# BraveGroup/DCD

Hardware: AMD Instinct MI355X
Metric: images/sec DGDE train step (bs=8, 384x1280) (higher is better)
Workload: dtype f32; 1 GPU; DGDE train bs=8 fp32 on 1xMI355X, synthetic KITTI 384x1280 + random kpts_ann (DGDE.yaml, DLA-34+DCNv2, 6 objects/image); global_batch=8, per_gpu_batch=8, input=384x1280, parallelism=dp1, dcn_precision=f32, step_launch=eager, sync_bn=False

## Files before the change

### dcd_amd/csrc/conv.hip

```cpp
#include <hip/hip_runtime.h>
#include <stdint.h>
#include <stdlib.h>

#include "../../include/dcd_hip.h"
#include "tuning_env.h"
#include "lds_limit.h"
#include "bf16_split.h"

typedef float f32x16 __attribute__((ext_vector_type(16)));
typedef float f32x4 __attribute__((ext_vector_type(4)));
typedef float f32x2 __attribute__((ext_vector_type(2)));

namespace {

constexpr int WN_CH = 8;
constexpr int WN_NT = 512;

template <int TR, int TC, int NB>
struct WinoGeom {
    static constexpr int KS = 32 * NB;
    static constexpr int U = 16 * KS * WN_CH;
    static constexpr int NTILE = TR * TC;
    static constexpr int ROWS = 4 * TR + 2;
    static constexpr int Q = (2 * TC + 8) / 4;
    static constexpr int RS = TC == 16 ? 48 : 42;
    static constexpr int PLANE = ROWS * RS;
    static constexpr int IN = WN_CH * PLANE;
    static constexpr int BUF = IN + U;
    static_assert(NTILE <= 32 && 4 * Q <= RS && RS % 2 == 0 && (2 * TC) % 4 == 0, "region geometry");
};

__device__ __forceinline__ void win_read4(const float *e, float (&q)[4])
{
    const f32x2 a = *reinterpret_cast<const f32x2 *>(e), b = *reinterpret_cast<const f32x2 *>(e + 2),
                c = *reinterpret_cast<const f32x2 *>(e + 4);
    q[0] = a.y; q[1] = b.x; q[2] = b.y; q[3] = c.x;
}

template <int RS>
__device__ __forceinline__ void win_store4(float *d, const f32x4 v)
{
    if constexpr (RS % 4 == 0) {
        *reinterpret_cast<f32x4 *>(d) = v;
    } else {
        *reinterpret_cast<f32x2 *>(d) = f32x2{v.x, v.y};
        *reinterpret_cast<f32x2 *>(d + 2) = f32x2{v.z, v.w};
    }
}

__device__ __forceinline__ void xcd_remap(int &bx, int &by)
{
    const int gx = gridDim.x, NT = gx * gridDim.y;
    const int L = bx + gx * by;
    const int xc = L & 7, slot = L >> 3;
    const int q = NT >> 3, r = NT & 7;
    const int Lp = (xc < r ? xc * (q + 1) : r * (q + 1) + (xc - r) * q) + slot;
    by = Lp / gx;
    bx = Lp - by * gx;
}

__device__ __forceinline__ void wino_prep_body(const float *__restrict__ w, float *__restrict__ ul, int Cc, int Kk, int mode, int nchunk,
                                               int nz, int WN_KS, int first, int step)
{
    const int n = nz * nchunk * WN_KS * WN_CH;
    for (int idx = first; idx < n; idx += step) {
        int r = idx;
        const int s = r & 3; r >>= 2;
        const int h = r & 1; r >>= 1;
        const int kk = r % WN_KS; r /= WN_KS;
        const int ck = r % nchunk, z = r / nchunk;
        const int k = z * WN_KS + kk, c = ck * WN_CH + 2 * s + h;
        float g[3][3];
#pragma unroll
        for (int a = 0; a < 3; ++a)
#pragma unroll
            for (int b = 0; b < 3; ++b) {
                float v = 0.f;
                if (k < Kk && c < Cc)
                    v = mode == 0 ? w[(((size_t)k * Cc + c) * 3 + a) * 3 + b] : w[(((size_t)c * Kk + k) * 3 + (2 - a)) * 3 + (2 - b)];
                g[a][b] = v;
            }
        float t[4][3];
#pragma unroll
        for (int b = 0; b < 3; ++b) {
            t[0][b] = g[0][b];
            t[1][b] = 0.5f * (g[0][b] + g[1][b] + g[2][b]);
            t[2][b] = 0.5f * (g[0][b] - g[1][b] + g[2][b]);
            t[3][b] = g[2][b];
        }
#pragma unroll
        for (int xi = 0; xi < 4; ++xi) {
            const float u[4] = {t[xi][0], 0.5f * (t[xi][0] + t[xi][1] + t[xi][2]), 0.5f * (t[xi][0] - t[xi][1] + t[xi][2]), t[xi][2]};
#pragma unroll
            for (int nu = 0; nu < 4; ++nu)
                ul[((((size_t)(z * nchunk + ck) * 16 + xi * 4 + nu) * 2 + h) * WN_KS + kk) * 4 + s] = u[nu];
        }
    }
}

__global__ void wino_prep_weights(const float *__restrict__ w, float *__restrict__ ul, int Cc, int Kk, int mode, int nchunk, int nz,
                                  int WN_KS)
{
    wino_prep_body(w, ul, Cc, Kk, mode, nchunk, nz, WN_KS, blockIdx.x * blockDim.x + threadIdx.x, gridDim.x * blockDim.x);
}

struct PrepBoth {
    float *ul[2];
    int Cc[2], Kk[2], nchunk[2], nz[2], ks[2];
};

__global__ void wino_prep_weights_both(const float *__restrict__ w, PrepBoth p)
{
    const int mode = blockIdx.y;
    if (!p.ul[mode]) return;
    wino_prep_body(w, p.ul[mode], p.Cc[mode], p.Kk[mode], mode, p.nchunk[mode], p.nz[mode], p.ks[mode],
                   blockIdx.x * blockDim.x + threadIdx.x, gridDim.x * blockDim.x);
}

__global__ void wino_prep_weights_table(const long long *__restrict__ table)
{
    const long long *e = table + 5 * (size_t)blockIdx.z;
    const float *w = reinterpret_cast<const float *>(e[0]);
    const int mode = blockIdx.y;
    float *ul = reinterpret_cast<float *>(e[1 + mode]);
    if (!w || !ul) return;
    const int Cin = (int)e[3], Cout = (int)e[4];
    const int Cc = mode ? Cout : Cin, Kk = mode ? Cin : Cout;
    const int WN_KS = Kk <= 32 ? 32 : 64;
    wino_prep_body(w, ul, Cc, Kk, mode, (Cc + WN_CH - 1) / WN_CH, (Kk + WN_KS - 1) / WN_KS, WN_KS,
                   blockIdx.x * blockDim.x + threadIdx.x, gridDim.x * blockDim.x);
}

template <int TR, int TC, int NB>
__global__ __launch_bounds__(WN_NT) void wino_conv3x3_f32(const float *__restrict__ x, const float *__restrict__ ul, float *y,
                                                          float *__restrict__ part, const float *__restrict__ bias,
                                                          const float *residual, int Cc, int H, int W, int Kk, int tiles_x,
                                                          int nchunk, int nz)
{
    using G = WinoGeom<TR, TC, NB>;
    constexpr int WN_ROWS = G::ROWS, WN_RS = G::RS, WN_PLANE = G::PLANE, WN_IN = G::IN, WN_BUF = G::BUF, WN_Q = G::Q;
    constexpr int WN_KS = G::KS, WN_U = G::U;
    extern __shared__ __attribute__((aligned(16))) float lds[];
    const int tid = threadIdx.x;
    const int lane = tid & 63, wave = tid >> 6;
    const int p = lane & 31, h = lane >> 5;
    const int xi = wave & 3, tg = wave >> 2;
    int bx = blockIdx.x, b = blockIdx.y;
    xcd_remap(bx, b);
    const int ty = bx / tiles_x, tx = bx - ty * tiles_x;
    const int r0 = ty * (4 * TR), c0 = tx * (2 * TC);
    const int z = blockIdx.z % nz, ks = blockIdx.z / nz, ksplit = gridDim.z / nz;
    const int ck0 = (int)((int64_t)ks * nchunk / ksplit), ck1 = (int)((int64_t)(ks + 1) * nchunk / ksplit);
    const int HW = H * W;
    const bool live = p < G::NTILE;
    const int pe = live ? p : 0;
    const int trow = pe / TC, tcol = pe - trow * TC;

    const int ra = xi == 0 ? 0 : 1, rb = xi == 3 ? 3 : 2;
    const float sa = xi == 2 ? -1.f : 1.f, sb = (xi == 0 || xi == 3) ? -1.f : 1.f;
    const int lanebase = (2 * TR * tg + 2 * trow) * WN_RS + 2 + 2 * tcol + h * WN_PLANE;
    const int base1 = lanebase + ra * WN_RS, base2 = lanebase + rb * WN_RS;

    const float *x_b = x + (size_t)b * Cc * HW;
    const float *ul_z = ul + (size_t)z * nchunk * WN_U;

    constexpr int KIN = (WN_CH * WN_ROWS * WN_Q + WN_NT - 1) / WN_NT;
    constexpr int KW = WN_U / 4 / WN_NT;
    int sg[KIN], sl[KIN];
    bool sv_[KIN];
#pragma unroll
    for (int k = 0; k < KIN; ++k) {
        const int e = tid + WN_NT * k;
        const int ch = e / (WN_ROWS * WN_Q), rem = e - ch * (WN_ROWS * WN_Q);
        const int row = rem / WN_Q, q = rem - row * WN_Q;
        const int yy = r0 - 1 + row, xx = c0 - 4 + 4 * q;
        sv_[k] = e < WN_CH * WN_ROWS * WN_Q;
        sg[k] = (sv_[k] && yy >= 0 && yy < H && xx >= 0 && xx < W) ? ch * HW + yy * W + xx : -1;
        sl[k] = ch * WN_PLANE + row * WN_RS + 4 * q;
    }
    f32x4 rin[KIN];
    auto issue_w = [&](int ck, float *buf) {
        const float *src = ul_z + (size_t)ck * WN_U + 4 * tid;
        float *dst = buf + WN_IN + 4 * 64 * __builtin_amdgcn_readfirstlane(wave);
#pragma unroll
        for (int k = 0; k < KW; ++k)
            __builtin_amdgcn_global_load_lds(src + 4 * WN_NT * k, (__attribute__((address_space(3))) void *)(dst + 4 * WN_NT * k), 16, 0, 0);
    };
    auto issue = [&](int ck) {
        const float *src = x_b + (size_t)ck * WN_CH * HW;
        const int cleft = Cc - ck * WN_CH;
#pragma unroll
        for (int k = 0; k < KIN; ++k) {
            const f32x4 zero4 = {0.f, 0.f, 0.f, 0.f};
            rin[k] = zero4;
            if (sv_[k] && sg[k] >= 0 && (tid + WN_NT * k) / (WN_ROWS * WN_Q) < cleft) rin[k] = *reinterpret_cast<const f32x4 *>(src + sg[k]);
        }
    };
    auto commit = [&](float *buf) {
#pragma unroll
        for (int k = 0; k < KIN; ++k)
            if (sv_[k]) win_store4<WN_RS>(buf + sl[k], rin[k]);
    };

    f32x16 acc[4][NB];
#pragma unroll
    for (int nu = 0; nu < 4; ++nu)
#pragma unroll
        for (int mb = 0; mb < NB; ++mb)
#pragma unroll
            for (int r = 0; r < 16; ++r) acc[nu][mb][r] = 0.f;

    issue_w(ck0, lds);
    issue(ck0);
    commit(lds);
    asm volatile("s_waitcnt vmcnt(0)" ::: "memory");
    __syncthreads();

    for (int ck = ck0; ck < ck1; ++ck) {
        const float *buf = lds + ((ck - ck0) & 1) * WN_BUF;
#ifndef WN_ABL_NOSTAGE
        if (ck + 1 < ck1) {
            issue_w(ck + 1, lds + ((ck + 1 - ck0) & 1) * WN_BUF);
            issue(ck + 1);
        }
#endif
        const float *ub = buf + WN_IN + ((xi * 4 * 2 + h) * WN_KS + p) * 4;
        const float *cp1 = buf + base1, *cp2 = buf + base2;
        f32x4 a0[4], a1[4];
#pragma unroll
        for (int nu = 0; nu < 4; ++nu) {
            a0[nu] = *reinterpret_cast<const f32x4 *>(ub + (nu * WN_KS) * 8);
            if (NB == 2) a1[nu] = *reinterpret_cast<const f32x4 *>(ub + (nu * WN_KS) * 8 + 32 * 4);
        }
        float qa[4], qb[4];
#ifndef WN_ABL_NOLDS
        win_read4(cp1, qa);
        win_read4(cp2, qb);
#endif
#pragma unroll
        for (int s = 0; s < 4; ++s) {
#ifdef WN_ABL_NOLDS
            const float t0 = sa * (float)s, t1 = sb, t2 = sa + sb, t3 = (float)ck;
#else
            const float t0 = sa * qa[0] + sb * qb[0], t1 = sa * qa[1] + sb * qb[1];
            const float t2 = sa * qa[2] + sb * qb[2], t3 = sa * qa[3] + sb * qb[3];
            if (s + 1 < 4) {
                win_read4(cp1 + 2 * (s + 1) * WN_PLANE, qa);
                win_read4(cp2 + 2 * (s + 1) * WN_PLANE, qb);
            }
#endif
            const float v[4] = {t0 - t2, t1 + t2, t2 - t1, t1 - t3};
            __builtin_amdgcn_sched_barrier(0);
#pragma unroll
            for (int nu = 0; nu < 4; ++nu) {
                acc[nu][0] = __builtin_amdgcn_mfma_f32_32x32x2f32(a0[nu][s], v[nu], acc[nu][0], 0, 0, 0);
                if (NB == 2) acc[nu][NB - 1] = __builtin_amdgcn_mfma_f32_32x32x2f32(a1[nu][s], v[nu], acc[nu][NB - 1], 0, 0, 0);
            }
        }
#ifndef WN_ABL_NOSTAGE
        if (ck + 1 < ck1) commit(lds + ((ck + 1 - ck0) & 1) * WN_BUF);
#endif
        asm volatile("s_waitcnt vmcnt(0)" ::: "memory");
        __syncthreads();
    }
#ifdef WN_ABL_NOEPI
    if (acc[0][0][0] != 123.456f) return;
#endif

    float *ex = lds;
    float *y_b = (ks == 0 ? y : part + (size_t)(ks - 1) * gridDim.y * Kk * HW) + (size_t)b * Kk * HW;
    const float *r_b = (residual && ks == 0) ? residual + (size_t)b * Kk * HW : nullptr;
    const int orow0 = r0 + 2 * TR * tg + 2 * trow, ocol = c0 + 2 * tcol;
#pragma unroll
    for (int mb = 0; mb < NB; ++mb) {
        float *mine = ex + (size_t)wave * 32 * 64 + lane;
#pragma unroll
        for (int r = 0; r < 16; ++r) {
            mine[r * 64] = acc[0][mb][r] + acc[1][mb][r] + acc[2][mb][r];
            mine[(16 + r) * 64] = acc[1][mb][r] - acc[2][mb][r] - acc[3][mb][r];
        }
        __syncthreads();
        const float *t0 = ex + (size_t)(tg * 4 + 0) * 32 * 64 + lane, *t1 = t0 + 32 * 64, *t2 = t1 + 32 * 64, *t3 = t2 + 32 * 64;
        if (live && ocol < W) {
#pragma unroll
            for (int rr = 0; rr < 4; ++rr) {
                const int r = 4 * xi + rr;
                const int k = z * WN_KS + mb * 32 + (r & 3) + 8 * (r >> 2) + 4 * h;
                const float a0 = t0[r * 64], a1 = t1[r * 64], a2 = t2[r * 64], a3 = t3[r * 64];
                const float b0 = t0[(16 + r) * 64], b1 = t1[(16 + r) * 64], b2 = t2[(16 + r) * 64], b3 = t3[(16 + r) * 64];
                if (k < Kk) {
                    const float bk = (bias && ks == 0) ? bias[k] : 0.f;
                    const size_t o = (size_t)k * HW + (size_t)orow0 * W + ocol;
                    float *dst = y_b + o;
                    f32x2 r0 = {bk, bk}, r1 = {bk, bk};
                    if (r_b) {
                        if (orow0 < H) r0 += *reinterpret_cast<const f32x2 *>(r_b + o);
                        if (orow0 + 1 < H) r1 += *reinterpret_cast<const f32x2 *>(r_b + o + W);
                    }
                    if (orow0 < H) *reinterpret_cast<f32x2 *>(dst) = f32x2{a0 + a1 + a2 + r0.x, b0 + b1 + b2 + r0.y};
                    if (orow0 + 1 < H) *reinterpret_cast<f32x2 *>(dst + W) = f32x2{a1 - a2 - a3 + r1.x, b1 - b2 - b3 + r1.y};
                }
            }
        }
        __syncthreads();
    }
}

constexpr int WS_CH = 16;

template <int NB>
__device__ __forceinline__ void wino_prep_split_body(const float *__restrict__ w, unsigned *__restrict__ us, int Cc, int Kk, int mode,
                                                     int nchunk, int nz, int first, int step)
{
    constexpr int KS = 32 * NB;
    const int n = nz * nchunk * KS * 2 * 4;
    for (int idx = first; idx < n; idx += step) {
        int r = idx;
        const int d = r & 3; r >>= 2;
        const int h = r & 1; r >>= 1;
        const int kk = r % KS; r /= KS;
        const int ck = r % nchunk, z = r / nchunk;
        const int k = z * KS + kk;
        float u[2][16];
#pragma unroll
        for (int e = 0; e < 2; ++e) {
            const int c = ck * WS_CH + 2 * (2 * d + e) + h;
            float g[3][3];
#pragma unroll
            for (int a = 0; a < 3; ++a)
#pragma unroll
                for (int b = 0; b < 3; ++b) {
                    float v = 0.f;
                    if (k < Kk && c < Cc)
                        v = mode == 0 ? w[(((size_t)k * Cc + c) * 3 + a) * 3 + b] : w[(((size_t)c * Kk + k) * 3 + (2 - a)) * 3 + (2 - b)];
                    g[a][b] = v;
                }
            float t[4][3];
#pragma unroll
            for (int b = 0; b < 3; ++b) {
                t[0][b] = g[0][b];
                t[1][b] = 0.5f * (g[0][b] + g[1][b] + g[2][b]);
                t[2][b] = 0.5f * (g[0][b] - g[1][b] + g[2][b]);
                t[3][b] = g[2][b];
            }
#pragma unroll
            for (int xi = 0; xi < 4; ++xi) {
                u[e][xi * 4 + 0] = t[xi][0];
                u[e][xi * 4 + 1] = 0.5f * (t[xi][0] + t[xi][1] + t[xi][2]);
                u[e][xi * 4 + 2] = 0.5f * (t[xi][0] - t[xi][1] + t[xi][2]);
                u[e][xi * 4 + 3] = t[xi][2];
            }
        }
        const int ob = kk >> 5, lane = h * 32 + (kk & 31);
        unsigned *dst = us + (size_t)(z * nchunk + ck) * (16 * NB * 2 * 256);
#pragma unroll
        for (int pos = 0; pos < 16; ++pos) {
            unsigned hi, lo;
            sp_split_pair(u[0][pos], u[1][pos], hi, lo);
            dst[((pos * NB + ob) * 2 + 0) * 256 + lane * 4 + d] = hi;
            dst[((pos * NB + ob) * 2 + 1) * 256 + lane * 4 + d] = lo;
        }
    }
}

#include "conv_direct_bf16.inc"
#include "conv1x1_bf16.inc"
#include "conv1x1_f32.inc"
#include "conv_s2_f32.inc"

template <int NB>
__global__ void wino_prep_weights_split(const float *__restrict__ w, unsigned *__restrict__ us, int Cc, int Kk, int mode, int nchunk,
                                        int nz)
{
    wino_prep_split_body<NB>(w, us, Cc, Kk, mode, nchunk, nz, blockIdx.x * blockDim.x + threadIdx.x, gridDim.x * blockDim.x);
}

__global__ void wino_prep_weights_split_table(const long long *__restrict__ table)
{
    const long long *e = table + 5 * (size_t)blockIdx.z;
    const float *w = reinterpret_cast<const float *>(e[0]);
    const int mode = blockIdx.y;
    unsigned *us = reinterpret_cast<unsigned *>(e[1 + mode]);
    if (!w || !us) return;
    const int Cin = (int)e[3], Cout = (int)e[4];
    const int Cc = mode ? Cout : Cin, Kk = mode ? Cin : Cout;
    const int nb = Kk <= 32 ? 1 : 2, nchunk = (Cc + WS_CH - 1) / WS_CH, nz = (Kk + 32 * nb - 1) / (32 * nb);
    const int first = blockIdx.x * blockDim.x + threadIdx.x, step = gridDim.x * blockDim.x;
    if (nb == 2) wino_prep_split_body<2>(w, us, Cc, Kk, mode, nchunk, nz, first, step);
    else wino_prep_split_body<1>(w, us, Cc, Kk, mode, nchunk, nz, first, step);
}

template <int NB, int NP>
__global__ __launch_bounds__(WN_NT) void wino_conv3x3_split(const float *__restrict__ x, const unsigned *__restrict__ us, float *y,
                                                            float *__restrict__ part, const float *__restrict__ bias,
                                                            const float *residual, int Cc, int H, int W, int Kk, int tiles_x,
                                                            int nchunk, int nz)
{
    constexpr int TR = 2, TC = 16;
    using G = WinoGeom<TR, TC, NB>;
    constexpr int WN_ROWS = G::ROWS, WN_RS = G::RS, WN_PLANE = G::PLANE, WN_Q = G::Q, WN_KS = G::KS;
    constexpr int WIN = (WS_CH * WN_PLANE + 3) & ~3;
    constexpr int WSLAB = 16 * NB * 2 * 256;
    extern __shared__ __attribute__((aligned(16))) float lds[];
    float *win = lds;
    unsigned *wbuf = reinterpret_cast<unsigned *>(lds + WIN);
    const int tid = threadIdx.x;
    const int lane = tid & 63, wave = __builtin_amdgcn_readfirstlane(tid >> 6);
    const int p = lane & 31, h = lane >> 5;
    const int xi = wave & 3, tg = wave >> 2;
    int bx = blockIdx.x, b = blockIdx.y;
    xcd_remap(bx, b);
    const int ty = bx / tiles_x, tx = bx - ty * tiles_x;
    const int r0 = ty * (4 * TR), c0 = tx * (2 * TC);
    const int z = blockIdx.z % nz, ks = blockIdx.z / nz, ksplit = gridDim.z / nz;
    const int ck0 = (int)((int64_t)ks * nchunk / ksplit), ck1 = (int)((int64_t)(ks + 1) * nchunk / ksplit);
    const int HW = H * W;
    const int trow = p / TC, tcol = p - trow * TC;

    const int ra = xi == 0 ? 0 : 1, rb = xi == 3 ? 3 : 2;
    const float sa = xi == 2 ? -1.f : 1.f, sb = (xi == 0 || xi == 3) ? -1.f : 1.f;
    const int lanebase = (2 * TR * tg + 2 * trow) * WN_RS + 2 + 2 * tcol + h * WN_PLANE;
    const int base1 = lanebase + ra * WN_RS, base2 = lanebase + rb * WN_RS;

    const float *x_b = x + (size_t)b * Cc * HW;
    const unsigned *us_z = us + (size_t)z * nchunk * WSLAB;

    constexpr int NITEM = WS_CH * WN_ROWS * WN_Q;
    constexpr int KIN = (NITEM + WN_NT - 1) / WN_NT;
    int sg[KIN], sl[KIN];
#pragma unroll
    for (int k = 0; k < KIN; ++k) {
        const int e = tid + WN_NT * k;
        const int ch = e / (WN_ROWS * WN_Q), rem = e - ch * (WN_ROWS * WN_Q);
        const int row = rem / WN_Q, q = rem - row * WN_Q;
        const int yy = r0 - 1 + row, xx = c0 - 4 + 4 * q;
        const bool ok = e < NITEM && yy >= 0 && yy < H && xx >= 0 && xx < W;
        sg[k] = ok ? ch * HW + yy * W + xx : -1;
        sl[k] = e < NITEM ? ch * WN_PLANE + row * WN_RS + 4 * q : -1;
    }
    f32x4 rin[KIN];
    auto issue_in = [&](int ck) {
        const float *src = x_b + (size_t)ck * WS_CH * HW;
        const int cleft = Cc - ck * WS_CH;
#pragma unroll
        for (int k = 0; k < KIN; ++k) {
            const f32x4 zero4 = {0.f, 0.f, 0.f, 0.f};
            rin[k] = zero4;
            if (sg[k] >= 0 && (tid + WN_NT * k) / (WN_ROWS * WN_Q) < cleft) rin[k] = *reinterpret_cast<const f32x4 *>(src + sg[k]);
        }
    };
    auto commit_in = [&]() {
#pragma unroll
        for (int k = 0; k < KIN; ++k)
// ... 291 lines not shown
    if (t0 < t1) {
        issue(t0);
        commit(lds);
        if (t0 + 1 < t1) issue(t0 + 1);
    }
    __syncthreads();
    for (int t = t0; t < t1; ++t) {
        const float *bw = lds + ((t - t0) & 1) * WW_BUF;
        float *nb = lds + (((t - t0) & 1) ^ 1) * WW_BUF;
        const float *ia = bw + lane_in + ra * WW_IROW, *ib = bw + lane_in + rb * WW_IROW;
        const float *d0 = bw + WW_IN + lane_dy, *d1 = d0 + (NOB - 1) * 32 * WW_DPLANE;
#ifdef WW_ABL_NOLDS
        float u0 = sa, u1 = sb;
#else
        const f32x2 pa0 = *reinterpret_cast<const f32x2 *>(ia), pa1 = *reinterpret_cast<const f32x2 *>(ia + 2);
        const f32x2 pb0 = *reinterpret_cast<const f32x2 *>(ib), pb1 = *reinterpret_cast<const f32x2 *>(ib + 2);
        f32x2 ca = *reinterpret_cast<const f32x2 *>(ia + 4), cb2 = *reinterpret_cast<const f32x2 *>(ib + 4);
        float u0 = sa * pa0.y + sb * pb0.y, u1 = sa * pa1.x + sb * pb1.x;
        float qa2 = pa1.y, qa3 = ca.x, qb2 = pb1.y, qb3 = cb2.x;
        f32x2 g00 = *reinterpret_cast<const f32x2 *>(d0), g01 = *reinterpret_cast<const f32x2 *>(d0 + 32);
        f32x2 g10 = *reinterpret_cast<const f32x2 *>(d1), g11 = *reinterpret_cast<const f32x2 *>(d1 + 32);
#endif
        float ev[12];
        sp_u32x2 pk[12];
#pragma unroll
        for (int s = 0; s < 8; ++s) {
#ifndef WW_ABL_NOSTAGE
            if (s == 4 && t + 1 < t1) {
                commit(nb);
                if (t + 2 < t1) issue(t + 2);
            }
#endif
#ifdef WW_ABL_NOLDS
            const float u2 = sa + (float)t, u3 = sb * (float)s;
            const float a0 = ea * (float)t, a1 = eb, b0 = ea + (float)s, b1 = eb * (float)s;
#else
            const float u2 = sa * qa2 + sb * qb2, u3 = sa * qa3 + sb * qb3;
            const float a0 = ea * g00.x + eb * g01.x, a1 = ea * g00.y + eb * g01.y;
            const float b0 = ea * g10.x + eb * g11.x, b1 = ea * g10.y + eb * g11.y;
            if (s + 1 < 8) {
                qa2 = ca.y; qb2 = cb2.y;
                ca = *reinterpret_cast<const f32x2 *>(ia + 2 * s + 6); cb2 = *reinterpret_cast<const f32x2 *>(ib + 2 * s + 6);
                qa3 = ca.x; qb3 = cb2.x;
                g00 = *reinterpret_cast<const f32x2 *>(d0 + 2 * s + 2); g01 = *reinterpret_cast<const f32x2 *>(d0 + 2 * s + 34);
                g10 = *reinterpret_cast<const f32x2 *>(d1 + 2 * s + 2); g11 = *reinterpret_cast<const f32x2 *>(d1 + 2 * s + 34);
            }
#endif
            const float v[4] = {u0 - u2, u1 + u2, u2 - u1, u1 - u3};
            const float wa[4] = {a0, a0 + a1, a0 - a1, -a1};
            const float wb[4] = {b0, b0 + b1, b0 - b1, -b1};
            if constexpr (BF) {
#pragma unroll
                for (int nu = 0; nu < 4; ++nu) {
                    if (s & 1) {
                        pk[nu][(s >> 1) & 1] = __builtin_bit_cast(unsigned, __builtin_convertvector(sp_f32x2{ev[nu], v[nu]}, sp_bf16x2));
                        pk[4 + nu][(s >> 1) & 1] = __builtin_bit_cast(unsigned, __builtin_convertvector(sp_f32x2{ev[4 + nu], wa[nu]}, sp_bf16x2));
                        if (NOB == 2) pk[8 + nu][(s >> 1) & 1] = __builtin_bit_cast(unsigned, __builtin_convertvector(sp_f32x2{ev[8 + nu], wb[nu]}, sp_bf16x2));
                    } else {
                        ev[nu] = v[nu]; ev[4 + nu] = wa[nu]; ev[8 + nu] = wb[nu];
                    }
                }
                if ((s & 3) == 3) {
#pragma unroll
                    for (int nu = 0; nu < 4; ++nu) {
                        const sp_s16x4 bv = __builtin_bit_cast(sp_s16x4, pk[nu]);
                        acc[nu][0] = __builtin_amdgcn_mfma_f32_32x32x8bf16_1k(__builtin_bit_cast(sp_s16x4, pk[4 + nu]), bv, acc[nu][0], 0, 0, 0);
                        if (NOB == 2)
                            acc[nu][NOB - 1] = __builtin_amdgcn_mfma_f32_32x32x8bf16_1k(__builtin_bit_cast(sp_s16x4, pk[8 + nu]), bv, acc[nu][NOB - 1], 0, 0, 0);
                    }
                }
            } else {
                __builtin_amdgcn_sched_barrier(0);
#pragma unroll
                for (int nu = 0; nu < 4; ++nu) {
                    acc[nu][0] = __builtin_amdgcn_mfma_f32_32x32x2f32(wa[nu], v[nu], acc[nu][0], 0, 0, 0);
                    if (NOB == 2) acc[nu][NOB - 1] = __builtin_amdgcn_mfma_f32_32x32x2f32(wb[nu], v[nu], acc[nu][NOB - 1], 0, 0, 0);
                }
            }
            u0 = u2;
            u1 = u3;
        }

#ifndef WW_ABL_NOBAR
        __syncthreads();
#endif
    }

#ifdef WW_ABL_NOEPI
    if (acc[0][0][0] != 123.456f) return;
#endif
    float *mine = part + ((size_t)blk * S + split) * WW_PART;
#pragma unroll
    for (int ob = 0; ob < NOB; ++ob)
#pragma unroll
        for (int r = 0; r < 16; ++r) {
            const int k = 32 * ob + (r & 3) + 8 * (r >> 2) + 4 * h;
            const float m0 = acc[0][ob][r], m1 = acc[1][ob][r], m2 = acc[2][ob][r], m3 = acc[3][ob][r];
            float *dst = mine + ((xi * 3) * KO + k) * 64 + cb * 32 + p;
            dst[0] = m0 + 0.5f * (m1 + m2);
            dst[KO * 64] = 0.5f * (m1 - m2);
            dst[2 * KO * 64] = 0.5f * (m1 + m2) + m3;
        }
}

__global__ __launch_bounds__(256) void wino_wrw_reduce(const float *__restrict__ part, float *__restrict__ gw, int Cin, int Cout, int S,
                                                       int ncg, int KO)
{
    __shared__ float m[12][17];
    const int tid = threadIdx.x;
    const int pos = tid >> 4, l = tid & 15;
    const int gidx = blockIdx.x * 16 + l;
    const int per = KO * 64;
    const int blk = gidx / per, kc = gidx - blk * per;
    if (pos < 12) {
        const float *src = part + ((size_t)blk * S * 12 + pos) * per + kc;
        float sum = 0.f;
#pragma unroll 8
        for (int sp = 0; sp < S; ++sp) sum += src[(size_t)sp * 12 * per];
        m[pos][l] = sum;
    }
    __syncthreads();
    if (pos < 9) {
        const int a = pos / 3, b = pos - a * 3;
        const float ga[4] = {a == 0 ? 1.f : 0.f, 0.5f, a == 1 ? -0.5f : 0.5f, a == 2 ? 1.f : 0.f};
        float r = 0.f;
#pragma unroll
        for (int xi = 0; xi < 4; ++xi) r += ga[xi] * m[xi * 3 + b][l];
        const int og = blk / ncg, cg = blk - og * ncg;
        const int k = og * KO + (kc >> 6), c = cg * 64 + (kc & 63);
        if (k < Cout && c < Cin) gw[((size_t)k * Cin + c) * 9 + pos] = r;
    }
}

}

struct ConvPlan {
    int geom;
    int nb;
    int tiles_x, tiles_y, nchunk, nz, ksplit;
};

static int device_cus()
{
    static int cus = 0;
    if (!cus) {
        int dev = 0, n = 0;
        if (hipGetDevice(&dev) != hipSuccess || hipDeviceGetAttribute(&n, hipDeviceAttributeMultiprocessorCount, dev) != hipSuccess || n <= 0)
            n = 256;
        cus = n;
    }
    return cus;
}

static ConvPlan conv_plan(int B, int Cc, int H, int W, int Kk)
{
    ConvPlan best{};
    const int cus = device_cus();
    int64_t best_cost = -1;
    for (int g = 0; g < 2; ++g) {
        ConvPlan p;
        p.geom = g;
        p.tiles_x = g == 0 ? (W + 31) / 32 : (W + 19) / 20;
        p.tiles_y = g == 0 ? (H + 7) / 8 : (H + 11) / 12;
        p.nchunk = (Cc + WN_CH - 1) / WN_CH;
        p.nb = Kk <= 32 ? 1 : 2;
        p.nz = (Kk + 32 * p.nb - 1) / (32 * p.nb);
        const int64_t wgs = (int64_t)p.tiles_x * p.tiles_y * B * p.nz;
        static const int min_chunks = dcd_env("DCD_CONV_MINCHUNK") ? atoi(dcd_env("DCD_CONV_MINCHUNK")) : 4;
        int ks = 1;
        while (ks < 8 && wgs * (ks * 2) <= cus && p.nchunk / (ks * 2) >= min_chunks) ks *= 2;
        p.ksplit = ks;
        const int64_t rounds = (wgs * ks + cus - 1) / cus;
        const int64_t cost = rounds * ((p.nchunk + ks - 1) / ks + 2) * (g == 0 ? 16 : 17);
        if (best_cost < 0 || cost < best_cost) {
            best_cost = cost;
            best = p;
        }
    }
    return best;
}

template <int TR, int TC, int NB>
static int conv_launch(hipStream_t stream, const ConvPlan &pl, const float *input, const float *ul, float *output, float *part,
                       const float *bias, const float *residual, int B, int Cc, int H, int W, int Kk)
{
    static LdsLimit lds_limit;
    size_t ldsb = (size_t)2 * WinoGeom<TR, TC, NB>::BUF * sizeof(float);
    if (ldsb < (size_t)8 * 32 * 64 * sizeof(float)) ldsb = (size_t)8 * 32 * 64 * sizeof(float);
    if (!lds_limit.raise((int)ldsb, wino_conv3x3_f32<TR, TC, NB>)) return DCD_ERR_LAUNCH;
    hipLaunchKernelGGL((wino_conv3x3_f32<TR, TC, NB>), dim3(pl.tiles_x * pl.tiles_y, B, pl.nz * pl.ksplit), dim3(WN_NT), ldsb, stream,
                       input, ul, output, part, bias, residual, Cc, H, W, Kk, pl.tiles_x, pl.nchunk, pl.nz);
    return DCD_OK;
}

template <int NB, int NP>
static int conv_launch_split(hipStream_t stream, const ConvPlan &pl, const float *input, const unsigned *us, float *output, float *part,
                             const float *bias, const float *residual, int B, int Cc, int H, int W, int Kk)
{
    static LdsLimit lds_limit;
    using G = WinoGeom<2, 16, NB>;
    const size_t ldsb = ((size_t)((WS_CH * G::PLANE + 3) & ~3) + (size_t)2 * 16 * NB * 2 * 256) * sizeof(float);
    if (!lds_limit.raise((int)ldsb, wino_conv3x3_split<NB, NP>)) return DCD_ERR_LAUNCH;
    hipLaunchKernelGGL((wino_conv3x3_split<NB, NP>), dim3(pl.tiles_x * pl.tiles_y, B, pl.nz * pl.ksplit), dim3(WN_NT), ldsb, stream, input,
                       us, output, part, bias, residual, Cc, H, W, Kk, pl.tiles_x, pl.nchunk, pl.nz);
    return DCD_OK;
}

static ConvPlan conv_plan_split(int B, int Cc, int H, int W, int Kk)
{
    ConvPlan p;
    p.geom = 0;
    p.tiles_x = (W + 31) / 32;
    p.tiles_y = (H + 7) / 8;
    p.nchunk = (Cc + WS_CH - 1) / WS_CH;
    p.nb = Kk <= 32 ? 1 : 2;
    p.nz = (Kk + 32 * p.nb - 1) / (32 * p.nb);
    const int64_t wgs = (int64_t)p.tiles_x * p.tiles_y * B * p.nz;
    const int cus = device_cus();
    int ks = 1;
    while (ks < 8 && wgs * (ks * 2) <= cus && p.nchunk / (ks * 2) >= 2) ks *= 2;
    p.ksplit = ks;
    return p;
}

static bool conv_direct_ok(int Cc, int H, int W)
{
    return (int64_t)(Cc + DC_CH) * H * W < (1ll << 29);
}

static ConvPlan conv_plan_direct(int B, int Cc, int H, int W, int Kk)
{
    static const int pin = dcd_env("DCD_CONV_DIRECT_P") ? atoi(dcd_env("DCD_CONV_DIRECT_P")) : 0;
    const int cus = device_cus();
    ConvPlan best{};
    int64_t best_cost = -1;
    for (int P = 2; P <= 4; P += 2) {
        if (P != (pin == 4 ? 4 : 2)) continue;
        ConvPlan p;
        static const int wxpin = dcd_env("DCD_CONV_DIRECT_WX") ? atoi(dcd_env("DCD_CONV_DIRECT_WX")) : 0;
        const int wx = P == 2 && wxpin == 2 ? 2 : 1;
        p.geom = P | (wx << 4);
        p.tiles_x = (W + 32 * wx - 1) / (32 * wx);
        p.tiles_y = (H + 4 * P - 1) / (4 * P);
        p.nchunk = (Cc + DC_CH - 1) / DC_CH;
        p.nb = Kk <= 32 ? 1 : 2;
        p.nz = (Kk + 32 * p.nb - 1) / (32 * p.nb);
        const int64_t wgs = (int64_t)p.tiles_x * p.tiles_y * B * p.nz;
        static const int min_chunks = dcd_env("DCD_CONV_DIRECT_MINCHUNK") ? atoi(dcd_env("DCD_CONV_DIRECT_MINCHUNK")) : 16;
        int ks = 1;
        while (ks < 8) {
            const int64_t next = wgs * ks * 2;
            const int left = p.nchunk / (ks * 2);
            const bool fill = next <= 3 * cus && left >= min_chunks;
            const bool small = 2 * next <= 3 * cus && left >= 2;
            if (!fill && !small) break;
            ks *= 2;
        }
        p.ksplit = ks;
        best = p;
    }
    (void)best_cost;
    return best;
}

template <int NB, int P, int MODE, int WX>
static int conv_launch_direct(hipStream_t stream, const ConvPlan &pl, const float *input, const unsigned *wd, float *output, float *part,
                              const float *bias, const float *residual, int B, int Cc, int H, int W, int Kk)
{
    static LdsLimit lds_limit;
    const size_t ldsb = ((size_t)2 * (4 * P + 2) * (32 * WX + 8) + (size_t)2 * 9 * NB * 64) * 16;
    if constexpr (MODE == 2) {
        if (!lds_limit.raise((int)ldsb, conv3x3_direct_bf16_w4<NB, P, WX>)) return DCD_ERR_LAUNCH;
        hipLaunchKernelGGL((conv3x3_direct_bf16_w4<NB, P, WX>), dim3(pl.tiles_x * pl.tiles_y, B, pl.nz * pl.ksplit), dim3(DC_NT * WX), ldsb,
                           stream, input, wd, output, part, bias, residual, Cc, H, W, Kk, pl.tiles_x, pl.nchunk, pl.nz);
    } else {
        if (!lds_limit.raise((int)ldsb, conv3x3_direct_bf16<NB, P, MODE, WX>)) return DCD_ERR_LAUNCH;
        hipLaunchKernelGGL((conv3x3_direct_bf16<NB, P, MODE, WX>), dim3(pl.tiles_x * pl.tiles_y, B, pl.nz * pl.ksplit), dim3(DC_NT * WX), ldsb,
                           stream, input, wd, output, part, bias, residual, Cc, H, W, Kk, pl.tiles_x, pl.nchunk, pl.nz);
    }
    return DCD_OK;
}

static size_t tw_dwords_split(int Cin, int Cout, int backward_data)
{
    const int Cc = backward_data ? Cout : Cin, Kk = backward_data ? Cin : Cout;
    const int nb = Kk <= 32 ? 1 : 2;
    return (size_t)((Cc + WS_CH - 1) / WS_CH) * ((Kk + 32 * nb - 1) / (32 * nb)) * 16 * nb * 2 * 256;
}

extern "C" {

size_t dcd_conv3x3_workspace_bytes(int B, int Cin, int H, int W, int Cout)
{
    if (B <= 0 || Cin <= 0 || Cout <= 0 || H <= 0 || W <= 0) return 0;
    const int cmax = Cin > Cout ? Cin : Cout;
    const size_t nchunk = (size_t)(cmax + WN_CH - 1) / WN_CH, nz = (size_t)(cmax + 63) / 64;
    const ConvPlan f = conv_plan(B, Cin, H, W, Cout), d = conv_plan(B, Cout, H, W, Cin);
    const size_t pf = (size_t)(f.ksplit - 1) * B * Cout * H * W, pd = (size_t)(d.ksplit - 1) * B * Cin * H * W;
    return (nchunk * nz * 16 * 64 * WN_CH + (pf > pd ? pf : pd)) * sizeof(float);
}

static int conv3x3_run(hipStream_t stream, const float *input, const float *weights, int prepared, const float *bias,
                       const float *residual, float *output, int B, int Cin, int H, int W, int Cout, int backward_data, void *workspace,
                       size_t workspace_bytes)
{
    (void)hipGetLastError();
    if (!input || !weights || !output || B <= 0 || Cin <= 0 || Cout <= 0 || H <= 0 || W <= 0) return DCD_ERR_BAD_ARG;
    if ((W & 3) || (H & 1) || (int64_t)(Cin > Cout ? Cin : Cout) * H * W >= (1ll << 31) || (bias && backward_data)) return DCD_ERR_BAD_ARG;
    const int Cc = backward_data ? Cout : Cin, Kk = backward_data ? Cin : Cout;
    ConvPlan pl = conv_plan(B, Cc, H, W, Kk);
    if (const char *e = dcd_env("DCD_CONV_GEOM")) {
        const int g = atoi(e);
        if (g == 0 || g == 1) {
            ConvPlan q = pl;
            q.geom = g;
            q.tiles_x = g == 0 ? (W + 31) / 32 : (W + 19) / 20;
            q.tiles_y = g == 0 ? (H + 7) / 8 : (H + 11) / 12;
            q.ksplit = 1;
            pl = q;
        }
    }
    const int ksz = 32 * pl.nb;
    const size_t ul_floats = prepared ? 0 : (size_t)pl.nchunk * pl.nz * 16 * ksz * WN_CH;
    const size_t img = (size_t)B * Kk * H * W;
    const size_t need = (ul_floats + (size_t)(pl.ksplit - 1) * img) * sizeof(float);
    if (need && (!workspace || workspace_bytes < need)) return DCD_ERR_WORKSPACE;
    float *part = (float *)workspace + ul_floats;
    const float *ul = weights;
    if (!prepared) {
        const int nprep = pl.nz * pl.nchunk * ksz * WN_CH;
        hipLaunchKernelGGL(wino_prep_weights, dim3((nprep + 255) / 256 < 4096 ? (nprep + 255) / 256 : 4096), dim3(256), 0, stream, weights,
                           (float *)workspace, Cc, Kk, backward_data ? 1 : 0, pl.nchunk, pl.nz, ksz);
        ul = (const float *)workspace;
    }
    const int st = pl.geom == 0 ? (pl.nb == 2 ? conv_launch<2, 16, 2>(stream, pl, input, ul, output, part, bias, residual, B, Cc, H, W, Kk)
                                              : conv_launch<2, 16, 1>(stream, pl, input, ul, output, part, bias, residual, B, Cc, H, W, Kk))
                                : (pl.nb == 2 ? conv_launch<3, 10, 2>(stream, pl, input, ul, output, part, bias, residual, B, Cc, H, W, Kk)
                                              : conv_launch<3, 10, 1>(stream, pl, input, ul, output, part, bias, residual, B, Cc, H, W, Kk));
    if (st != DCD_OK) return st;
    if (pl.ksplit > 1) {
        const size_t n4 = img / 4;
        const int nb = (int)((n4 + 255) / 256 < 2048 ? (n4 + 255) / 256 : 2048);
        hipLaunchKernelGGL(wino_sum_partials, dim3(nb), dim3(256), 0, stream, output, (const float *)part, n4, pl.ksplit - 1);
    }
    return hipGetLastError() == hipSuccess ? DCD_OK : DCD_ERR_LAUNCH;
}

int dcd_conv3x3(void *stream_, const float *input, const float *weight, const float *bias, const float *residual, float *output,
                int B, int Cin, int H, int W, int Cout, int backward_data, void *workspace, size_t workspace_bytes)
{
    if (!workspace) return DCD_ERR_BAD_ARG;
    return conv3x3_run((hipStream_t)stream_, input, weight, 0, bias, residual, output, B, Cin, H, W, Cout, backward_data, workspace,
                       workspace_bytes);
}

static size_t tw_floats(int Cin, int Cout, int backward_data)
{
    const int Cc = backward_data ? Cout : Cin, Kk = backward_data ? Cin : Cout;
    const int nb = Kk <= 32 ? 1 : 2, ks = 32 * nb;
    return (size_t)((Cc + WN_CH - 1) / WN_CH) * ((Kk + ks - 1) / ks) * 16 * ks * WN_CH;
}

size_t dcd_conv3x3_weights_bytes(int Cin, int Cout, int backward_data)
{
    return Cin > 0 && Cout > 0 ? tw_floats(Cin, Cout, backward_data) * sizeof(float) : 0;
}

int dcd_conv3x3_transform_weights(void *stream_, const float *weight, int Cin, int Cout, float *forward_out, float *backward_out)
{
    (void)hipGetLastError();
    if (!weight || Cin <= 0 || Cout <= 0 || (!forward_out && !backward_out)) return DCD_ERR_BAD_ARG;
    PrepBoth p;
    int nmax = 0;
    for (int mode = 0; mode < 2; ++mode) {
        const int Cc = mode ? Cout : Cin, Kk = mode ? Cin : Cout;
        p.ul[mode] = mode ? backward_out : forward_out;
        p.Cc[mode] = Cc;
        p.Kk[mode] = Kk;
        p.ks[mode] = Kk <= 32 ? 32 : 64;
        p.nchunk[mode] = (Cc + WN_CH - 1) / WN_CH;
        p.nz[mode] = (Kk + p.ks[mode] - 1) / p.ks[mode];
        const int n = p.nz[mode] * p.nchunk[mode] * p.ks[mode] * WN_CH;
        if (p.ul[mode] && n > nmax) nmax = n;
    }
    const int nb = (nmax + 255) / 256 < 4096 ? (nmax + 255) / 256 : 4096;
    hipLaunchKernelGGL(wino_prep_weights_both, dim3(nb, 2), dim3(256), 0, (hipStream_t)stream_, weight, p);
    return hipGetLastError() == hipSuccess ? DCD_OK : DCD_ERR_LAUNCH;
}

int dcd_conv3x3_transform_weights_table(void *stream_, const long long *table, int entries)
{
    (void)hipGetLastError();
    if (!table || entries <= 0 || entries > 65535) return DCD_ERR_BAD_ARG;
    hipLaunchKernelGGL(wino_prep_weights_table, dim3(64, 2, entries), dim3(256), 0, (hipStream_t)stream_, table);
    return hipGetLastError() == hipSuccess ? DCD_OK : DCD_ERR_LAUNCH;
}

int dcd_conv3x3_prepared(void *stream_, const float *input, const float *transformed, const float *bias, const float *residual,
                         float *output, int B, int Cin, int H, int W, int Cout, int backward_data, void *workspace,
                         size_t workspace_bytes)
{
    return conv3x3_run((hipStream_t)stream_, input, transformed, 1, bias, residual, output, B, Cin, H, W, Cout, backward_data, workspace,
                       workspace_bytes);
}

size_t dcd_conv3x3_split_weights_bytes(int Cin, int Cout, int backward_data)
{
    return Cin > 0 && Cout > 0 ? tw_dwords_split(Cin, Cout, backward_data) * sizeof(unsigned) : 0;
}

int dcd_conv3x3_split_transform_weights(void *stream_, const float *weight, int Cin, int Cout, void *forward_out, void *backward_out)
{
    hipStream_t stream = (hipStream_t)stream_;
    (void)hipGetLastError();
    if (!weight || Cin <= 0 || Cout <= 0 || (!forward_out && !backward_out)) return DCD_ERR_BAD_ARG;
    for (int mode = 0; mode < 2; ++mode) {
        unsigned *dst = (unsigned *)(mode ? backward_out : forward_out);
        if (!dst) continue;
        const int Cc = mode ? Cout : Cin, Kk = mode ? Cin : Cout;
        const int nb = Kk <= 32 ? 1 : 2, nchunk = (Cc + WS_CH - 1) / WS_CH, nz = (Kk + 32 * nb - 1) / (32 * nb);
        const int n = nz * nchunk * 32 * nb * 8;
        const int grid = (n + 255) / 256 < 4096 ? (n + 255) / 256 : 4096;
        if (nb == 2) hipLaunchKernelGGL(wino_prep_weights_split<2>, dim3(grid), dim3(256), 0, stream, weight, dst, Cc, Kk, mode, nchunk, nz);
        else hipLaunchKernelGGL(wino_prep_weights_split<1>, dim3(grid), dim3(256), 0, stream, weight, dst, Cc, Kk, mode, nchunk, nz);
    }
    return hipGetLastError() == hipSuccess ? DCD_OK : DCD_ERR_LAUNCH;
}

int dcd_conv3x3_split_transform_weights_table(void *stream_, const long long *table, int entries)
{
    (void)hipGetLastError();
    if (!table || entries <= 0 || entries > 65535) return DCD_ERR_BAD_ARG;
    hipLaunchKernelGGL(wino_prep_weights_split_table, dim3(64, 2, entries), dim3(256), 0, (hipStream_t)stream_, table);
    return hipGetLastError() == hipSuccess ? DCD_OK : DCD_ERR_LAUNCH;
}

size_t dcd_conv3x3_split_workspace_bytes(int B, int Cin, int H, int W, int Cout)
{
    if (B <= 0 || Cin <= 0 || Cout <= 0 || H <= 0 || W <= 0) return 0;
    const ConvPlan f = conv_plan_split(B, Cin, H, W, Cout), d = conv_plan_split(B, Cout, H, W, Cin);
    const size_t pf = (size_t)(f.ksplit - 1) * B * Cout * H * W, pd = (size_t)(d.ksplit - 1) * B * Cin * H * W;
    return (pf > pd ? pf : pd) * sizeof(float) + 16;
}

int dcd_conv3x3_split_prepared(void *stream_, const float *input, const void *transformed, const float *bias, const float *residual,
                               float *output, int B, int Cin, int H, int W, int Cout, int backward_data, int precision, void *workspace,
                               size_t workspace_bytes)
{
    hipStream_t stream = (hipStream_t)stream_;
    (void)hipGetLastError();
    if (!input || !transformed || !output || B <= 0 || Cin <= 0 || Cout <= 0 || H <= 0 || W <= 0) return DCD_ERR_BAD_ARG;
    if (precision != DCD_PREC_BF16X3 && precision != DCD_PREC_BF16) return DCD_ERR_BAD_ARG;
    const bool one = precision == DCD_PREC_BF16;
    if ((W & 3) || (H & 1) || (int64_t)(Cin > Cout ? Cin : Cout) * H * W >= (1ll << 31) || (bias && backward_data)) return DCD_ERR_BAD_ARG;
    const int Cc = backward_data ? Cout : Cin, Kk = backward_data ? Cin : Cout;
    const ConvPlan pl = conv_plan_split(B, Cc, H, W, Kk);
    const size_t img = (size_t)B * Kk * H * W;
    const size_t need = (size_t)(pl.ksplit - 1) * img * sizeof(float);
    if (need && (!workspace || workspace_bytes < need)) return DCD_ERR_WORKSPACE;
    float *part = (float *)workspace;
    const unsigned *us = (const unsigned *)transformed;
    const int st = pl.nb == 2 ? (one ? conv_launch_split<2, 1>(stream, pl, input, us, output, part, bias, residual, B, Cc, H, W, Kk)
                                     : conv_launch_split<2, 3>(stream, pl, input, us, output, part, bias, residual, B, Cc, H, W, Kk))
                              : (one ? conv_launch_split<1, 1>(stream, pl, input, us, output, part, bias, residual, B, Cc, H, W, Kk)
                                     : conv_launch_split<1, 3>(stream, pl, input, us, output, part, bias, residual, B, Cc, H, W, Kk));
    if (st != DCD_OK) return st;
    if (pl.ksplit > 1) {
        const size_t n4 = img / 4;
        const int nb = (int)((n4 + 255) / 256 < 2048 ? (n4 + 255) / 256 : 2048);
        hipLaunchKernelGGL(wino_sum_partials, dim3(nb), dim3(256), 0, stream, output, (const float *)part, n4, pl.ksplit - 1);
    }
    return hipGetLastError() == hipSuccess ? DCD_OK : DCD_ERR_LAUNCH;
}

size_t dcd_conv3x3_bf16_weights_bytes(int Cin, int Cout, int backward_data)
{
    if (Cin <= 0 || Cout <= 0) return 0;
    return 16 * (backward_data ? dc_weight_slots(Cout, Cin) : dc_weight_slots(Cin, Cout));
}

int dcd_conv3x3_bf16_transform_weights(void *stream_, const float *weight, int Cin, int Cout, void *forward_out, void *backward_out)
{
    hipStream_t stream = (hipStream_t)stream_;
    (void)hipGetLastError();
    if (!weight || Cin <= 0 || Cout <= 0 || (!forward_out && !backward_out)) return DCD_ERR_BAD_ARG;
    DirectPrep p;
    size_t nmax = 0;
    for (int mode = 0; mode < 2; ++mode) {
        p.ud[mode] = (unsigned *)(mode ? backward_out : forward_out);
        p.Cc[mode] = mode ? Cout : Cin;
        p.Kk[mode] = mode ? Cin : Cout;
        const size_t n = p.ud[mode] ? dc_weight_slots(p.Cc[mode], p.Kk[mode]) : 0;
        if (n > nmax) nmax = n;
    }
    nmax /= 9;
    const int nb = (int)((nmax + 255) / 256 < 2048 ? (nmax + 255) / 256 : 2048);
    hipLaunchKernelGGL(direct_prep_weights_both, dim3(nb, 2), dim3(256), 0, stream, weight, p);
    return hipGetLastError() == hipSuccess ? DCD_OK : DCD_ERR_LAUNCH;
}

int dcd_conv3x3_bf16_transform_weights_table(void *stream_, const long long *table, int entries)
{
    (void)hipGetLastError();
    if (!table || entries <= 0 || entries > 65535) return DCD_ERR_BAD_ARG;
    hipLaunchKernelGGL(direct_prep_weights_table, dim3(32, 2, entries), dim3(256), 0, (hipStream_t)stream_, table);
    return hipGetLastError() == hipSuccess ? DCD_OK : DCD_ERR_LAUNCH;
}

size_t dcd_conv3x3_bf16_workspace_bytes(int B, int Cin, int H, int W, int Cout)
{
    if (B <= 0 || Cin <= 0 || Cout <= 0 || H <= 0 || W <= 0) return 0;
    const size_t pf = (size_t)(conv_plan_direct(B, Cin, H, W, Cout).ksplit - 1) * B * Cout * H * W;
    const size_t pd = (size_t)(conv_plan_direct(B, Cout, H, W, Cin).ksplit - 1) * B * Cin * H * W;
    return (pf > pd ? pf : pd) * sizeof(float) + 16;
}

int dcd_conv3x3_bf16_prepared(void *stream_, const float *input, const void *transformed, const float *bias, const float *residual,
                              float *output, int B, int Cin, int H, int W, int Cout, int backward_data, void *workspace,
                              size_t workspace_bytes)
{
    hipStream_t stream = (hipStream_t)stream_;
    (void)hipGetLastError();
    if (!input || !transformed || !output || B <= 0 || Cin <= 0 || Cout <= 0 || H <= 0 || W <= 0) return DCD_ERR_BAD_ARG;
    if (bias && backward_data) return DCD_ERR_BAD_ARG;
    const int Cc = backward_data ? Cout : Cin, Kk = backward_data ? Cin : Cout;
    if (!conv_direct_ok(Cc, H, W) || (int64_t)Kk * H * W >= (1ll << 31) || (W & 3)) return DCD_ERR_BAD_ARG;
    const ConvPlan pl = conv_plan_direct(B, Cc, H, W, Kk);
    const size_t img = (size_t)B * Kk * H * W;
    const size_t need = (size_t)(pl.ksplit - 1) * img * sizeof(float);
    if (need && (!workspace || workspace_bytes < need)) return DCD_ERR_WORKSPACE;
    if (pl.ksplit > 1 && (img & 3)) return DCD_ERR_BAD_ARG;
    float *part = (float *)workspace;
    const unsigned *wd = (const unsigned *)transformed;
    static const int mpin = dcd_env("DCD_CONV_DIRECT_MODE") ? atoi(dcd_env("DCD_CONV_DIRECT_MODE")) : -1;
    const int P = pl.geom & 15, wx = pl.geom >> 4;
    const int mode = P == 4 ? 0 : (mpin >= 0 ? mpin : 1);
#define DCD_DIRECT(NB_, P_, M_, WX_) conv_launch_direct<NB_, P_, M_, WX_>(stream, pl, input, wd, output, part, bias, residual, B, Cc, H, W, Kk)
#define DCD_DIRECT_NB(NB_)                                                                                                              \
    (P == 4 ? DCD_DIRECT(NB_, 4, 0, 1)                                                                                                  \
            : wx == 2 ? (mode == 2 ? DCD_DIRECT(NB_, 2, 2, 2) : DCD_DIRECT(NB_, 2, 1, 2))                                               \
                      : (mode == 2 ? DCD_DIRECT(NB_, 2, 2, 1) : mode == 1 ? DCD_DIRECT(NB_, 2, 1, 1) : DCD_DIRECT(NB_, 2, 0, 1)))
    const int st = pl.nb == 2 ? DCD_DIRECT_NB(2) : DCD_DIRECT_NB(1);
#undef DCD_DIRECT_NB
#undef DCD_DIRECT
    if (st != DCD_OK) return st;
    if (pl.ksplit > 1) {
        const size_t n4 = img / 4;
// ... 274 lines not shown
```

Before: 215.3 images/s.

## Use single-block Winograd tiles for thin convs, hint occupancy, prefetch residual

```diff
diff --git a/dcd_amd/csrc/conv.hip b/dcd_amd/csrc/conv.hip
--- a/dcd_amd/csrc/conv.hip
+++ b/dcd_amd/csrc/conv.hip
@@ -117,7 +117,12 @@
                    blockIdx.x * blockDim.x + threadIdx.x, gridDim.x * blockDim.x);
 }
 
-__global__ void wino_prep_weights_table(const long long *__restrict__ table)
+__host__ __device__ inline int wino_nb(int Cc, int Kk, bool thin)
+{
+    return Kk <= 32 || (thin && Cc <= 32) ? 1 : 2;
+}
+
+__global__ void wino_prep_weights_table(const long long *__restrict__ table, int thin)
 {
     const long long *e = table + 5 * (size_t)blockIdx.z;
     const float *w = reinterpret_cast<const float *>(e[0]);
@@ -126,16 +131,16 @@
     if (!w || !ul) return;
     const int Cin = (int)e[3], Cout = (int)e[4];
     const int Cc = mode ? Cout : Cin, Kk = mode ? Cin : Cout;
-    const int WN_KS = Kk <= 32 ? 32 : 64;
+    const int WN_KS = 32 * wino_nb(Cc, Kk, thin != 0);
     wino_prep_body(w, ul, Cc, Kk, mode, (Cc + WN_CH - 1) / WN_CH, (Kk + WN_KS - 1) / WN_KS, WN_KS,
                    blockIdx.x * blockDim.x + threadIdx.x, gridDim.x * blockDim.x);
 }
 
 template <int TR, int TC, int NB>
-__global__ __launch_bounds__(WN_NT) void wino_conv3x3_f32(const float *__restrict__ x, const float *__restrict__ ul, float *y,
-                                                          float *__restrict__ part, const float *__restrict__ bias,
-                                                          const float *residual, int Cc, int H, int W, int Kk, int tiles_x,
-                                                          int nchunk, int nz)
+__global__ __launch_bounds__(WN_NT) __attribute__((amdgpu_waves_per_eu(NB == 1 ? 4 : 2)))
+void wino_conv3x3_f32(const float *__restrict__ x, const float *__restrict__ ul, float *y, float *__restrict__ part,
+                      const float *__restrict__ bias, const float *residual, int Cc, int H, int W, int Kk, int tiles_x, int nchunk,
+                      int nz)
 {
     using G = WinoGeom<TR, TC, NB>;
     constexpr int WN_ROWS = G::ROWS, WN_RS = G::RS, WN_PLANE = G::PLANE, WN_IN = G::IN, WN_BUF = G::BUF, WN_Q = G::Q;
@@ -267,38 +272,67 @@
     if (acc[0][0][0] != 123.456f) return;
 #endif
 
+    int te = tid;
+    asm volatile("" : "+v"(te));
+    const int lane_e = te & 63, wave_e = te >> 6;
+    const int h_e = lane_e >> 5, xi_e = wave_e & 3, tg_e = wave_e >> 2;
+    const bool live_e = (lane_e & 31) < G::NTILE;
+    const int pe_e = live_e ? (lane_e & 31) : 0;
+    const int trow_e = pe_e / TC, tcol_e = pe_e - trow_e * TC;
     float *ex = lds;
     float *y_b = (ks == 0 ? y : part + (size_t)(ks - 1) * gridDim.y * Kk * HW) + (size_t)b * Kk * HW;
     const float *r_b = (residual && ks == 0) ? residual + (size_t)b * Kk * HW : nullptr;
-    const int orow0 = r0 + 2 * TR * tg + 2 * trow, ocol = c0 + 2 * tcol;
+    const int orow0 = r0 + 2 * TR * tg_e + 2 * trow_e, ocol = c0 + 2 * tcol_e;
+    const bool store = live_e && ocol < W;
 #pragma unroll
     for (int mb = 0; mb < NB; ++mb) {
-        float *mine = ex + (size_t)wave * 32 * 64 + lane;
+        f32x2 q0[4], q1[4];
+        float bk[4];
+        auto load_res = [&]() {
+#pragma unroll
+            for (int rr = 0; rr < 4; ++rr) {
+                const int r = 4 * xi_e + rr;
+                const int k = z * WN_KS + mb * 32 + (r & 3) + 8 * (r >> 2) + 4 * h_e;
+                bk[rr] = (bias && ks == 0 && store && k < Kk) ? bias[k] : 0.f;
+                q0[rr] = f32x2{0.f, 0.f};
+                q1[rr] = f32x2{0.f, 0.f};
+                if (r_b && store && k < Kk) {
+                    const size_t o = (size_t)k * HW + (size_t)orow0 * W + ocol;
+                    if (orow0 < H) q0[rr] = *reinterpret_cast<const f32x2 *>(r_b + o);
+                    if (orow0 + 1 < H) q1[rr] = *reinterpret_cast<const f32x2 *>(r_b + o + W);
+                }
+            }
+        };
+#ifndef WN_ABL_LATE_RESIDUAL
+        load_res();
+#endif
+        float *mine = ex + (size_t)wave_e * 32 * 64 + lane_e;
 #pragma unroll
         for (int r = 0; r < 16; ++r) {
             mine[r * 64] = acc[0][mb][r] + acc[1][mb][r] + acc[2][mb][r];
             mine[(16 + r) * 64] = acc[1][mb][r] - acc[2][mb][r] - acc[3][mb][r];
         }
         __syncthreads();
-        const float *t0 = ex + (size_t)(tg * 4 + 0) * 32 * 64 + lane, *t1 = t0 + 32 * 64, *t2 = t1 + 32 * 64, *t3 = t2 + 32 * 64;
-        if (live && ocol < W) {
+#ifdef WN_ABL_LATE_RESIDUAL
+        load_res();
+#endif
+        const float *t0 = ex + (size_t)(tg_e * 4 + 0) * 32 * 64 + lane_e, *t1 = t0 + 32 * 64, *t2 = t1 + 32 * 64, *t3 = t2 + 32 * 64;
+        if (store) {
 #pragma unroll
             for (int rr = 0; rr < 4; ++rr) {
-                const int r = 4 * xi + rr;
-                const int k = z * WN_KS + mb * 32 + (r & 3) + 8 * (r >> 2) + 4 * h;
+                const int r = 4 * xi_e + rr;
+                const int k = z * WN_KS + mb * 32 + (r & 3) + 8 * (r >> 2) + 4 * h_e;
                 const float a0 = t0[r * 64], a1 = t1[r * 64], a2 = t2[r * 64], a3 = t3[r * 64];
                 const float b0 = t0[(16 + r) * 64], b1 = t1[(16 + r) * 64], b2 = t2[(16 + r) * 64], b3 = t3[(16 + r) * 64];
                 if (k < Kk) {
-                    const float bk = (bias && ks == 0) ? bias[k] : 0.f;
-                    const size_t o = (size_t)k * HW + (size_t)orow0 * W + ocol;
-                    float *dst = y_b + o;
-                    f32x2 r0 = {bk, bk}, r1 = {bk, bk};
+                    float *dst = y_b + (size_t)k * HW + (size_t)orow0 * W + ocol;
+                    f32x2 rv0 = {bk[rr], bk[rr]}, rv1 = rv0;
                     if (r_b) {
-                        if (orow0 < H) r0 += *reinterpret_cast<const f32x2 *>(r_b + o);
-                        if (orow0 + 1 < H) r1 += *reinterpret_cast<const f32x2 *>(r_b + o + W);
+                        rv0 += q0[rr];
+                        rv1 += q1[rr];
                     }
-                    if (orow0 < H) *reinterpret_cast<f32x2 *>(dst) = f32x2{a0 + a1 + a2 + r0.x, b0 + b1 + b2 + r0.y};
-                    if (orow0 + 1 < H) *reinterpret_cast<f32x2 *>(dst + W) = f32x2{a1 - a2 - a3 + r1.x, b1 - b2 - b3 + r1.y};
+                    if (orow0 < H) *reinterpret_cast<f32x2 *>(dst) = f32x2{a0 + a1 + a2 + rv0.x, b0 + b1 + b2 + rv0.y};
+                    if (orow0 + 1 < H) *reinterpret_cast<f32x2 *>(dst + W) = f32x2{a1 - a2 - a3 + rv1.x, b1 - b2 - b3 + rv1.y};
                 }
             }
         }
@@ -896,6 +930,17 @@
     return cus;
 }
 
+static bool conv_thin_nb()
+{
+    const char *e = dcd_env("DCD_CONV_THIN_NB");
+    return !(e && atoi(e) == 0);
+}
+
+static int conv_nb(int Cc, int Kk)
+{
+    return wino_nb(Cc, Kk, conv_thin_nb());
+}
+
 static ConvPlan conv_plan(int B, int Cc, int H, int W, int Kk)
 {
     ConvPlan best{};
@@ -907,7 +952,7 @@
         p.tiles_x = g == 0 ? (W + 31) / 32 : (W + 19) / 20;
         p.tiles_y = g == 0 ? (H + 7) / 8 : (H + 11) / 12;
         p.nchunk = (Cc + WN_CH - 1) / WN_CH;
-        p.nb = Kk <= 32 ? 1 : 2;
+        p.nb = conv_nb(Cc, Kk);
         p.nz = (Kk + 32 * p.nb - 1) / (32 * p.nb);
         const int64_t wgs = (int64_t)p.tiles_x * p.tiles_y * B * p.nz;
         static const int min_chunks = dcd_env("DCD_CONV_MINCHUNK") ? atoi(dcd_env("DCD_CONV_MINCHUNK")) : 4;
@@ -1101,7 +1146,7 @@
 static size_t tw_floats(int Cin, int Cout, int backward_data)
 {
     const int Cc = backward_data ? Cout : Cin, Kk = backward_data ? Cin : Cout;
-    const int nb = Kk <= 32 ? 1 : 2, ks = 32 * nb;
+    const int ks = 32 * conv_nb(Cc, Kk);
     return (size_t)((Cc + WN_CH - 1) / WN_CH) * ((Kk + ks - 1) / ks) * 16 * ks * WN_CH;
 }
 
@@ -1121,7 +1166,7 @@
         p.ul[mode] = mode ? backward_out : forward_out;
         p.Cc[mode] = Cc;
         p.Kk[mode] = Kk;
-        p.ks[mode] = Kk <= 32 ? 32 : 64;
+        p.ks[mode] = 32 * conv_nb(Cc, Kk);
         p.nchunk[mode] = (Cc + WN_CH - 1) / WN_CH;
         p.nz[mode] = (Kk + p.ks[mode] - 1) / p.ks[mode];
         const int n = p.nz[mode] * p.nchunk[mode] * p.ks[mode] * WN_CH;
@@ -1136,7 +1181,8 @@
 {
     (void)hipGetLastError();
     if (!table || entries <= 0 || entries > 65535) return DCD_ERR_BAD_ARG;
-    hipLaunchKernelGGL(wino_prep_weights_table, dim3(64, 2, entries), dim3(256), 0, (hipStream_t)stream_, table);
+    hipLaunchKernelGGL(wino_prep_weights_table, dim3(64, 2, entries), dim3(256), 0, (hipStream_t)stream_, table,
+                       conv_thin_nb() ? 1 : 0);
     return hipGetLastError() == hipSuccess ? DCD_OK : DCD_ERR_LAUNCH;
 }
 
```

Measured after the change: 214.5 images/s. No clear change (-0.4%).
